# SHI-Labs/SH-GAN

Measured on AMD Instinct MI355X. Metric: generator images/sec, higher is better.
Workload: dtype f32

## Files before the change

include/shgan_hip.h:

```cpp
#ifndef SHGAN_HIP_H
#define SHGAN_HIP_H
#include <stddef.h>
#include <stdint.h>
#ifdef __cplusplus
extern "C" {
#endif

#define SHG_OK 0
#define SHG_ERR_ARG (-1)
#define SHG_ERR_LAUNCH (-2)
#define SHG_ERR_UNSUPPORTED (-3)

int shg_abi_version(void);
const char* shg_last_error(void);
int shg_device_info(int dev, char* buf, int buflen);

int shg_upfirdn2d_out_size(int H, int W, int fh, int fw, int upx, int upy, int downx, int downy, int padx0, int padx1,
                           int pady0, int pady1, int* OH, int* OW);
int shg_upfirdn2d_f32(const float* x, const float* f, float* y, int N, int C, int H, int W, int fh, int fw, int upx, int upy,
                      int downx, int downy, int padx0, int padx1, int pady0, int pady1, int flip, float gain, void* stream);
int shg_upfirdn2d_strided(const void* x, const float* f, void* y, int dtype, int N, int C, int H, int W, const long* x_strides,
                          const long* y_strides, int fh, int fw, long f_stride_y, long f_stride_x, int upx, int upy, int downx, int downy,
                          int padx0, int padx1, int pady0, int pady1, int flip, float gain, void* stream);
int shg_upfirdn2d_epilogue_f32(const float* x, const float* f, float* y, int N, int C, int H, int W, int fh, int fw, int upx,
// ... 4 lines not shown
int shg_bias_act_f32(const float* x, float* y, const float* scale, const float* bias, const float* noise, int noise_mode,
                     float noise_strength, const float* residual, int N, int C, int HW, int act, float alpha, float gain,
                     float clamp, void* stream);
int shg_bias_act_backward_f32(const float* g, const float* y, float* dx, long total, int act, float alpha, float gain, float clamp,
                              void* stream);
int shg_fma_f32(const float* a, const float* b, const float* c, float* y, long total, void* stream);
int shg_fma_bcast(const void* a, const void* b, const void* c, void* y, int nd, const long* shape, const long* sa, const long* sb,
                  const long* sc, int f64, void* stream);
int shg_mul_reduce(const void* g, const void* b, void* out, int nd, int nk, const long* shape, const long* sg, const long* sb,
                   int inner_kept, int f64, void* stream);
int shg_scale_channels_f32(const float* x, const float* s, float* y, int NC, int HW, void* stream);
int shg_sum_partials_f32(const float* part, float* out, int N, int B, int K, void* stream);
int shg_scale_cast_f32_f16(const void* src, void* dst, long n, float gain, int to_half, void* stream);
int shg_planes_to_image_f32(const float* mid, const float* bias, float* y, int N, int C, int H, int W, int lo, int OH, int OW,
                            void* stream);

int shg_conv_weight_prep_f32(const float* w, float* wt, float* wscale, float* wsq, int O, int I, int KH, int KW, int OP,
                             int demod, float gain, int flip, void* stream);
int shg_conv2d_f32(const float* x, const float* wt, float* y, int NB, int I, int O, int OP, int H, int W, int kh, int kw,
                   int mode, int pad, int wgroups, long wstride, const float* in_scale, const float* out_scale,
                   const float* bias, const float* noise, int noise_mode, float noise_strength, int act, float alpha, float gain,
                   float clamp, const float* residual, int out_mode, void* workspace, size_t ws_bytes, void* stream);
size_t shg_conv2d_workspace_bytes(int NB, int I, int O, int H, int W, int kh, int kw, int mode, int pad, int wgroups);
int shg_conv_wino_chunk(void);
int shg_conv_weight_prep_wino_f32(const float* w, const float* wscale, float* wu, int O, int I, int OP, int flip, void* stream);
int shg_conv2d_wino_f32(const float* x, const float* wu, float* y, int NB, int I, int O, int OP, int H, int W,
                        const float* in_scale, const float* out_scale, const float* bias, const float* noise, int noise_mode,
                        float noise_strength, int act, float alpha, float gain, float clamp, const float* residual, void* stream);
size_t shg_conv2d_wino_workspace_bytes(int NB, int I, int O, int OP, int H, int W);
int shg_conv2d_wino_ws_f32(const float* x, const float* wu, float* y, int NB, int I, int O, int OP, int H, int W,
                           const float* in_scale, const float* out_scale, const float* bias, const float* noise, int noise_mode,
                           float noise_strength, int act, float alpha, float gain, float clamp, const float* residual, void* workspace,
                           size_t ws_bytes, void* stream);
long shg_conv_wino4_weight_elems(int OP, int I);
int shg_conv_weight_prep_wino4_f32(const float* w, const float* wscale, float* wu, int O, int I, int OP, int flip, void* stream);
int shg_conv2d_wino4_supported(int NB, int I, int O, int H, int W);
int shg_conv2d_wino4_f32(const float* x, const float* wu, float* y, int NB, int I, int O, int OP, int H, int W,
                         const float* in_scale, const float* out_scale, const float* bias, const float* noise, int noise_mode,
                         float noise_strength, int act, float alpha, float gain, float clamp, const float* residual, void* stream);
size_t shg_conv2d_wino4_workspace_bytes(int NB, int I, int O, int OP, int H, int W);
int shg_conv2d_wino4_ws_f32(const float* x, const float* wu, float* y, int NB, int I, int O, int OP, int H, int W,
                            const float* in_scale, const float* out_scale, const float* bias, const float* noise, int noise_mode,
                            float noise_strength, int act, float alpha, float gain, float clamp, const float* residual, void* workspace,
                            size_t ws_bytes, void* stream);
int shg_upfir_planar_f32(const float* mid, const float* f, float* y, int N, int C, int H, int W, int flip, float gain,
                         const float* scale, const float* bias, const float* noise, int noise_mode, float noise_strength,
// ... 163 lines not shown
```

sh-gan_amd/_lib.py:

```python
import ctypes
import os

import torch

_HERE = os.path.dirname(os.path.abspath(__file__))
LIB_PATH = os.path.join(_HERE, 'lib', 'libshgan_hip.so')
ABI_VERSION = 40

c_fp = ctypes.c_void_p
c_i = ctypes.c_int
c_f = ctypes.c_float
c_l = ctypes.c_long
c_pp = ctypes.POINTER(ctypes.c_void_p)



class DenseGroup(ctypes.Structure):
    _fields_ = [('x1', c_fp), ('x2', c_fp), ('w', c_fp), ('b', c_fp), ('y', c_fp),
                ('ld1', c_i), ('ld2', c_i), ('K1', c_i), ('K2', c_i), ('O', c_i), ('ldy', c_i),
                ('wgain', c_f), ('bgain', c_f)]


class StyleGroup(ctypes.Structure):
    _fields_ = [('styles', c_fp), ('wsq', c_fp), ('s_out', c_fp), ('dcoef', c_fp),
# ... 5 lines not shown
        (n, c_i) for n in ('I', 'H', 'W', 'x_ctot', 'x_coff', 'O', 'kh', 'kw', 'sh', 'sw', 'ph', 'pw', 'OH', 'OW', 'y_ctot', 'y_coff', 'splitk')]


_SIGS = {
    'shg_abi_version': [],
    'shg_device_info': [c_i, ctypes.c_char_p, c_i],
    'shg_upfirdn2d_out_size': [c_i] * 12 + [ctypes.POINTER(c_i), ctypes.POINTER(c_i)],
    'shg_upfirdn2d_f32': [c_fp, c_fp, c_fp] + [c_i] * 15 + [c_f, c_fp],
    'shg_upfirdn2d_strided': [c_fp, c_fp, c_fp, c_i, c_i, c_i, c_i, c_i, ctypes.POINTER(c_l), ctypes.POINTER(c_l), c_i, c_i, c_l, c_l] + [c_i] * 9
                             + [c_f, c_fp],
    'shg_upfirdn2d_epilogue_f32': [c_fp, c_fp, c_fp] + [c_i] * 15 + [c_f, c_fp, c_fp, c_fp, c_i, c_f, c_i, c_f, c_f, c_f, c_fp, c_fp],
    'shg_bias_act_f32': [c_fp, c_fp, c_fp, c_fp, c_fp, c_i, c_f, c_fp, c_i, c_i, c_i, c_i, c_f, c_f, c_f, c_fp],
    'shg_fma_f32': [c_fp, c_fp, c_fp, c_fp, c_l, c_fp],
    'shg_fma_bcast': [c_fp, c_fp, c_fp, c_fp, c_i] + [ctypes.POINTER(c_l)] * 4 + [c_i, c_fp],
    'shg_mul_reduce': [c_fp, c_fp, c_fp, c_i, c_i] + [ctypes.POINTER(c_l)] * 3 + [c_i, c_i, c_fp],
    'shg_scale_channels_f32': [c_fp, c_fp, c_fp, c_i, c_i, c_fp],
    'shg_sum_partials_f32': [c_fp, c_fp, c_i, c_i, c_i, c_fp],
    'shg_scale_cast_f32_f16': [c_fp, c_fp, c_l, c_f, c_i, c_fp],
    'shg_planes_to_image_f32': [c_fp, c_fp, c_fp, c_i, c_i, c_i, c_i, c_i, c_i, c_i, c_fp],
    'shg_conv_weight_prep_f32': [c_fp, c_fp, c_fp, c_fp, c_i, c_i, c_i, c_i, c_i, c_i, c_f, c_i, c_fp],
    'shg_conv2d_f32': [c_fp, c_fp, c_fp] + [c_i] * 11 + [c_l, c_fp, c_fp, c_fp, c_fp, c_i, c_f, c_i, c_f, c_f, c_f, c_fp, c_i,
                       c_fp, ctypes.c_size_t, c_fp],
    'shg_conv2d_workspace_bytes': [c_i] * 10,
    'shg_conv_wino_chunk': [],
    'shg_conv_weight_prep_wino_f32': [c_fp, c_fp, c_fp, c_i, c_i, c_i, c_i, c_fp],
    'shg_conv2d_wino_f32': [c_fp, c_fp, c_fp] + [c_i] * 6 + [c_fp, c_fp, c_fp, c_fp, c_i, c_f, c_i, c_f, c_f, c_f, c_fp, c_fp],
    'shg_conv2d_wino_ws_f32': [c_fp, c_fp, c_fp] + [c_i] * 6 + [c_fp, c_fp, c_fp, c_fp, c_i, c_f, c_i, c_f, c_f, c_f, c_fp, c_fp, ctypes.c_size_t, c_fp],
    'shg_conv2d_wino_workspace_bytes': [c_i] * 6,
    'shg_conv_wino4_weight_elems': [c_i, c_i],
    'shg_conv_weight_prep_wino4_f32': [c_fp, c_fp, c_fp, c_i, c_i, c_i, c_i, c_fp],
    'shg_conv2d_wino4_supported': [c_i] * 5,
    'shg_conv2d_wino4_f32': [c_fp, c_fp, c_fp] + [c_i] * 6 + [c_fp, c_fp, c_fp, c_fp, c_i, c_f, c_i, c_f, c_f, c_f, c_fp, c_fp],
    'shg_conv2d_wino4_ws_f32': [c_fp, c_fp, c_fp] + [c_i] * 6 + [c_fp, c_fp, c_fp, c_fp, c_i, c_f, c_i, c_f, c_f, c_f, c_fp, c_fp, ctypes.c_size_t, c_fp],
    'shg_conv2d_wino4_workspace_bytes': [c_i] * 6,
    'shg_upfir_planar_f32': [c_fp, c_fp, c_fp, c_i, c_i, c_i, c_i, c_i, c_f, c_fp, c_fp, c_fp, c_i, c_f, c_i, c_f, c_f, c_f, c_fp, c_fp],
    'shg_upfir_planar_sep_supported': [c_i, c_i],
    'shg_upfir_planar_sep_f32': [c_fp, ctypes.POINTER(c_f), c_fp, c_i, c_i, c_i, c_i, c_i, c_f, c_fp, c_fp, c_fp, c_i, c_f, c_i, c_f, c_f, c_f, c_fp, c_fp],
    'shg_conv1x1_thin_in_f32': [c_fp, c_fp, c_fp, c_fp, c_i, c_i, c_i, c_i, c_f, c_i, c_f, c_f, c_f, c_fp],
    'shg_torgb_f32': [c_fp, c_fp, c_fp, c_fp, c_fp, c_fp, c_fp, c_i, c_i, c_i, c_i, c_i, c_fp],
    'shg_dense_f32': [c_fp, c_fp, c_fp, c_fp, c_i, c_i, c_i, c_i, c_i, c_f, c_f, c_i, c_f, c_f, c_f, c_fp],
    'shg_demod_weight_f32': [c_fp, c_fp, c_fp, c_fp, c_i, c_i, c_i, c_i, c_fp],
    'shg_demod_weight_backward_f32': [c_fp, c_fp, c_fp, c_fp, c_fp, c_i, c_i, c_i, c_fp],
    'shg_style_factors_f32': [c_fp, c_fp, c_fp, c_fp, c_fp, c_i, c_i, c_i, c_i, c_fp],
    'shg_style_factors_backward_f32': [c_fp, c_fp, c_fp, c_fp, c_fp, c_fp, c_fp, c_fp, c_fp, c_i, c_i, c_i, c_i, c_fp],
    'shg_matmul_nn_f32': [c_fp, c_fp, c_fp, c_i, c_i, c_i, c_i, c_i, c_f, c_fp],
    'shg_matmul_tn_f32': [c_fp, c_fp, c_fp, c_fp, c_i, c_i, c_i, c_i, c_i, c_f, c_f, c_fp],
# ... 124 lines not shown
```

sh-gan_amd/csrc/conv_mfma.hip:

```cpp
#include "shg_device.h"
#include <stdlib.h>
#include <utility>

struct ConvParams {
    const float* x;
    const float* wt;
    float* y;
    float* part;
    const float* in_scale;
    const float* out_scale;
    const float* bias;
    const float* noise;
    const float* residual;
    int NB, I, O, OP;
    int IPK;
    int H, W;
    int OHp, OWp;
    int OHt, OWt;
    int S;
    int dy0, dx0;
    int span_y, span_x;
    struct TileClass {
        int n_tiles;
        int TW, TH, TN;
        int tiles_x, tiles_y;
        int oy_base, ox_base, rows, cols;
        int PH, PW, PATCH;
    } cls[3];
    int patch_max, tn_max;
    int n_ptiles, n_otiles;
    int wgroups;
    long wstride;
    int ksplit, i_per_slice;
    long part_stride;
    int out_mode;
    int noise_mode;
    float noise_strength;
    int act;
    float alpha, gain, clamp;
    int tap_off[9];
    int tail_first, tail_ks, tail_ips, fix;
    float* tail_ws;
    int raw_reduce;
};

template <class F, int... S>
__device__ __forceinline__ void static_for_impl(F&& f, std::integer_sequence<int, S...>) {
    (f(std::integral_constant<int, S>{}), ...);
}
template <int N, class F>
__device__ __forceinline__ void static_for(F&& f) {
    static_for_impl(static_cast<F&&>(f), std::make_integer_sequence<int, N>{});
}

__device__ __forceinline__ float conv_epilogue(const ConvParams& p, float v, int n, int o, long idx, float nz) {
    if (p.out_scale) v *= p.out_scale[n * p.O + o];
    v += nz;
    if (p.bias) v += p.bias[o];
    v = p.act ? shg_lrelu_agc(v, p.alpha, p.gain, p.clamp) : v * p.gain;
    if (p.residual) v += p.residual[idx];
    return v;
}

template <int NTAPS, int KC, int MO, int NP, int WO, int WP, int XQ, bool UP, bool DB, int OCC>
__global__ __launch_bounds__(WO * WP * 64, OCC) void conv_mfma_kernel(const ConvParams p) {
    constexpr int BO = MO * 32 * WO;
    constexpr int NT = WO * WP * 64;
    constexpr int ROWS = KC * NTAPS;
    constexpr int XP = KC + 1;
    constexpr int NPH = UP ? 4 : 1;
    constexpr int V4 = ROWS * BO / 4;
    constexpr int PER = (V4 + NT - 1) / NT;
    extern __shared__ __attribute__((aligned(16))) float smem[];
    constexpr int WSZ = ROWS * BO;
    constexpr int NBUF = DB ? 2 : 1;
    float* Wl = smem;
    float* Sl = smem + NBUF * WSZ;
    float* Xl = Sl + (p.in_scale ? p.tn_max * p.i_per_slice : 0);
    const int XSZ = XP * p.patch_max;

    const int tid = threadIdx.x;
    const int lane = tid & 63, wave = tid >> 6;
    const int l31 = lane & 31, half = lane >> 5;
    const int wo = wave / WP, wp = wave % WP;

    const int nwork = p.n_ptiles * p.n_otiles;
    int kslice, work, tslice = -1;
    if (p.fix) { kslice = 0; work = p.tail_first + blockIdx.x; }
// ... 95 lines not shown
                const int ic = g * 4 + c;
                xv[k][ic] = p.x[xo[k] + (unsigned)(min(i0 + ic, p.I - 1) * HW)];
            }
        }
    };
    auto piece_store = [&](int j, int i0, int buf) __attribute__((always_inline)) {
        if (j < PW0) {
            const int e = tid + j * NT;
            if (e < V4) *reinterpret_cast<f32x4*>(Wl + buf * WSZ + e * 4) = wv[j];
        } else {
            const int k = (j - PW0) / XG, g = (j - PW0) % XG;
            const int q = tid + k * NT;
            f32x4 sc = {1.f, 1.f, 1.f, 1.f};
            if (p.in_scale) sc = *reinterpret_cast<const f32x4*>(Sl + xsn[k] + (i0 - i_begin) + g * 4);
            if (q < PATCH) {
                float* dst = Xl + buf * XSZ + q * XP + g * 4;
#pragma unroll
                for (int c = 0; c < 4; ++c)
                    dst[c] = (xoff[k] >= 0 && i0 + g * 4 + c < i_end) ? xv[k][g * 4 + c] * sc[c] : 0.f;
            }
        }
    };

    auto w_dma = [&](int i0, int buf) __attribute__((always_inline)) {
#pragma unroll
        for (int k = 0; k < PER; ++k) {
            if ((k + 1) * NT <= V4 || k * NT + wave * 64 < V4)
                __builtin_amdgcn_global_load_lds((const __attribute__((address_space(1))) void*)(wbase + (size_t)i0 * NTAPS * 64 + wl[k]),
                                                 (__attribute__((address_space(3))) void*)(Wl + buf * WSZ + (k * NT + wave * 64) * 4), 16, 0, 0);
        }
    };
    if (!p.fix) {
        if (WDMA) w_dma(i_begin, 0);
#pragma unroll
        for (int j = 0; j < NPIECE; ++j) piece_load(j, i_begin);
        __syncthreads();
#pragma unroll
        for (int j = 0; j < NPIECE; ++j) piece_store(j, i_begin, 0);
        if (DB && i_begin + KC < i_end) {
#pragma unroll
            for (int j = 0; j < NPIECE; ++j) piece_load(j, i_begin + KC);
        }
        __syncthreads();
    }

    int cur = 0;
    for (int i0 = i_begin; i0 < i_end; i0 += KC, cur ^= (DB ? 1 : 0)) {
        const bool more = i0 + KC < i_end;
        const bool more2 = i0 + 2 * KC < i_end;
        if (WDMA && more) w_dma(i0 + KC, cur ^ 1);
        if (!DB && more) {
#pragma unroll
            for (int j = 0; j < NPIECE; ++j) piece_load(j, i0 + KC);
        }
        const float* wa_c = wa + cur * WSZ;
        const float* xb_c[NP];
#pragma unroll
        for (int np = 0; np < NP; ++np) xb_c[np] = xbase[np] + cur * XSZ;
        auto handover = [&]() __attribute__((always_inline)) {
            if (more) {
#pragma unroll
                for (int j = 0; j < NPIECE; ++j) piece_store(j, i0 + KC, cur ^ 1);
            }
            if (more2) {
#pragma unroll
                for (int j = 0; j < NPIECE; ++j) piece_load(j, i0 + 2 * KC);
            }
        };
        constexpr int NGRP = (DB && WO * WP >= 8) ? (WO * WP) / 4 : 1;
        const int grp = wave >> 2;

        if constexpr (!UP) {
            constexpr int NSTEP = NTAPS * (KC / 2);
            float a[2][MO], b[2][NP];
            auto fetch = [&](int step, int buf) __attribute__((always_inline)) {
                const int t = step / (KC / 2), c2 = step % (KC / 2);
                const int toff = p.tap_off[t] * XP;
#pragma unroll
                for (int mo = 0; mo < MO; ++mo) a[buf][mo] = wa_c[((c2 * 2) * NTAPS + t) * BO + mo * 32];
#pragma unroll
                for (int np = 0; np < NP; ++np) b[buf][np] = xb_c[np][toff + c2 * 2];
            };
            fetch(0, 0);
            auto step_body = [&](int step) __attribute__((always_inline)) {
                if (step + 1 < NSTEP) fetch(step + 1, (step + 1) & 1);
                __builtin_amdgcn_sched_barrier(0);
#pragma unroll
                for (int mo = 0; mo < MO; ++mo)
#pragma unroll
                    for (int np = 0; np < NP; ++np)
// ... 47 lines not shown
#pragma unroll
                        for (int np = 0; np < NP; ++np)
                            acc[PHASE[t]][mo][np] = __builtin_amdgcn_mfma_f32_32x32x2f32(
                                a[slot & 1][tt][mo], b[c2 & 1][SHIFT[t]][np], acc[PHASE[t]][mo][np], 0, 0, 0);
                }
            };
            static_for<NSLOT>([&](auto sc) __attribute__((always_inline)) {
                constexpr int slot = decltype(sc)::value;
                slot_body(slot);
                if constexpr (DB) {
                    static_for<NGRP>([&](auto gc) __attribute__((always_inline)) {
                        constexpr int g = decltype(gc)::value;
                        if constexpr (slot == ((2 * g + 1) * NSLOT) / (2 * NGRP)) {
                            __builtin_amdgcn_sched_barrier(0);
                            if (NGRP == 1 || grp == g) handover();
                            __builtin_amdgcn_sched_barrier(0);
                        }
                    });
                }
            });
        }
        __syncthreads();
        if (!DB && more) {
#pragma unroll
            for (int j = 0; j < NPIECE; ++j) piece_store(j, i0 + KC, 0);
            __syncthreads();
        }
    }

    constexpr int NREG = NPH * MO * NP * 16;
    float* const tws = (tslice >= 0 || p.fix)
        ? p.tail_ws + ((size_t)(work - p.tail_first) * p.tail_ks + (tslice >= 0 ? tslice : 0)) * NREG * NT + tid : nullptr;

#pragma unroll
    for (int np = 0; np < NP; ++np) {
        const int j = (wp * NP + np) * 32 + l31;
        const int tn = j / THW;
        const int rem = j - tn * THW;
        const int ty = rem / TW, tx = rem - ty * TW;
        const int n = n0 + tn, oy = oy0 + ty, ox = ox0 + tx;
        if (tn >= TN || n >= p.NB || oy >= oy_end || ox >= ox_end) continue;
#pragma unroll
        for (int ph = 0; ph < NPH; ++ph) {
            long plane = (long)p.OHt * p.OWt;
            long base;
            int pix;
            if constexpr (UP) {
                const int a = ph >> 1, b = ph & 1;
// ... 45 lines not shown
                        if (o < p.O) p.y[base + (long)o * plane] = acc[ph][mo][np][r] * p.gain;
                    }
                    continue;
                }
                float osc[16], bs[16], rs[16];
#pragma unroll
                for (int r = 0; r < 16; ++r) {
                    const int o = min(ob + (r & 3) + 8 * (r >> 2), p.O - 1);
                    osc[r] = p.out_scale ? p.out_scale[n * p.O + o] : 1.f;
                    bs[r] = p.bias ? p.bias[o] : 0.f;
                    rs[r] = p.residual ? p.residual[base + (long)o * plane] : 0.f;
                }
#pragma unroll
                for (int r = 0; r < 16; ++r) {
                    const int o = ob + (r & 3) + 8 * (r >> 2);
                    if (o >= p.O) continue;
                    float v = acc[ph][mo][np][r] * osc[r] + nz + bs[r];
                    v = p.act ? shg_lrelu_agc(v, p.alpha, p.gain, p.clamp) : v * p.gain;
                    p.y[base + (long)o * plane] = v + rs[r];
                }
            }
        }
    }
}

__global__ __launch_bounds__(256) void splitk_reduce_kernel(const ConvParams p, long total, long plane) {
    const long stride = (long)gridDim.x * 256;
    for (long e = (long)blockIdx.x * 256 + threadIdx.x; e < total; e += stride) {
        float v = 0.f;
        for (int s = 0; s < p.ksplit; ++s) v += p.part[(long)s * p.part_stride + e];
        if (p.raw_reduce) { p.y[e] = v; continue; }
        const long no = e / plane;
        const int pix = (int)(e - no * plane);
        const int n = (int)(no / p.O), o = (int)(no - (long)n * p.O);
        float nz = 0.f;
        if (p.noise_mode == 1) nz = p.noise[pix] * p.noise_strength;
        else if (p.noise_mode == 2) nz = p.noise[(long)n * plane + pix] * p.noise_strength;
        p.y[e] = conv_epilogue(p, v, n, o, e, nz);
    }
}



static void tile_search(ConvParams::TileClass& t, int NB, int rows, int cols, int BP, int wgroups, int S, int span_y, int span_x,
                        int patch_cap) {
    long best = -1, bpatch = 0;
// ... 38 lines not shown
    }
    p.n_ptiles = p.cls[0].n_tiles + p.cls[1].n_tiles + p.cls[2].n_tiles;
    p.n_otiles = shg_cdiv(p.O, BO);
    p.patch_max = 0; p.tn_max = 1;
    for (int i = 0; i < 3; ++i) {
        if (p.cls[i].n_tiles == 0) continue;
        if (p.cls[i].PATCH > p.patch_max) p.patch_max = p.cls[i].PATCH;
        if (p.cls[i].TN > p.tn_max) p.tn_max = p.cls[i].TN;
    }
}

static int conv_ksplit(int grid, int chunks, bool allow) {
    int ks = 1;
    if (allow) while (grid * ks < 512 && chunks / (ks * 2) >= 4 && ks < 64) ks *= 2;
    return ks;
}

static constexpr int CONV_UP_MIN = 16;

static int conv_cu_count() { return shg_cu_count(); }

static size_t conv_tail_ws_bound(bool up) { return (size_t)256 * (up ? 128 * 128 * 4 : 128 * 256) * sizeof(float); }

template <int NTAPS, int KC, int MO, int NP, int WO, int WP, int XQ, bool UP, bool DB, int OCC>
static int launch_conv(ConvParams& p, void* workspace, size_t ws_bytes, hipStream_t s) {
    constexpr int BO = MO * 32 * WO, BP = NP * 32 * WP, NT = WO * WP * 64;
    const long out_elems = (UP && p.out_mode == 1) ? 4L * p.NB * p.O * (p.H + 1) * (p.W + 1) : (long)p.NB * p.O * p.OHt * p.OWt;
    conv_tiles(p, BO, BP, UP, XQ * NT);
    const int chunks = shg_cdiv(p.I, KC);
    int ks = conv_ksplit(p.n_ptiles * p.n_otiles, chunks, workspace != nullptr);
    if (DB && p.n_ptiles * p.n_otiles >= conv_cu_count()) ks = 1;
    while (ks > 1 && (size_t)ks * out_elems * sizeof(float) > ws_bytes) ks /= 2;
    p.i_per_slice = shg_cdiv(chunks, ks) * KC;
    p.ksplit = shg_cdiv(p.I, p.i_per_slice);
    p.raw_reduce = UP ? 1 : 0;
    p.part = p.ksplit > 1 ? (float*)workspace : nullptr;
    p.part_stride = out_elems;
    if (p.patch_max > XQ * NT) { shg_set_error("conv: patch of %d elements exceeds the staging capacity %d", p.patch_max, XQ * NT); return SHG_ERR_UNSUPPORTED; }
    if (!UP)
        for (int t = 0; t < NTAPS; ++t) {
            const int dyr = p.tap_off[t] >> 6, dxr = p.tap_off[t] & 63;
            p.tap_off[t] = dyr * p.cls[0].PW + dxr;
        }
    const size_t lds = sizeof(float) * ((DB ? 2 : 1) * ((size_t)KC * NTAPS * BO + (size_t)(KC + 1) * p.patch_max) +
                                        (p.in_scale ? (size_t)p.tn_max * p.i_per_slice : 0));
    auto kern = conv_mfma_kernel<NTAPS, KC, MO, NP, WO, WP, XQ, UP, DB, OCC>;
    if (lds > 64 * 1024) {
        if (lds > 160 * 1024) { shg_set_error("conv: LDS request %zu exceeds 160 KiB", lds); return SHG_ERR_UNSUPPORTED; }
        hipError_t e = hipFuncSetAttribute(reinterpret_cast<const void*>(kern), hipFuncAttributeMaxDynamicSharedMemorySize, (int)lds);
        if (e != hipSuccess) { shg_set_error("hipFuncSetAttribute: %s", hipGetErrorString(e)); return SHG_ERR_LAUNCH; }
    }
    const int nwork = p.n_ptiles * p.n_otiles;
    p.tail_first = nwork; p.tail_ks = 1; p.tail_ips = p.I; p.fix = 0; p.tail_ws = nullptr;
    int n_tail = 0;
    if (DB && p.ksplit == 1 && workspace) {
        const int slots = conv_cu_count();
        const int tail = nwork % slots;
        if (nwork > slots && tail > 0 && tail * 10 < slots * 6) {
            int tk = 1;
            while (tk < 8 && tail * tk * 2 <= slots && chunks / (tk * 2) >= 4) tk *= 2;
            const size_t need = (size_t)tail * tk * (BO * BP * (UP ? 4 : 1)) * sizeof(float);
            if (tk > 1 && need <= ws_bytes) {
                n_tail = tail; p.tail_first = nwork - tail; p.tail_ks = tk; p.tail_ips = shg_cdiv(chunks, tk) * KC;
                p.tail_ws = (float*)workspace;
            }
        }
    }
    const int grid = p.ksplit > 1 ? nwork * p.ksplit : p.tail_first + n_tail * p.tail_ks;
    hipLaunchKernelGGL(kern, dim3(grid), dim3(NT), lds, s, p);
// ... 233 lines not shown
        const size_t split = ks > 1 ? (size_t)ks * 4 * NB * O * (H + 1) * (W + 1) * sizeof(float) : 0;
        const size_t tail = big ? conv_tail_ws_bound(true) : 0;
        return split > tail ? split : tail;
    }
    const int S = mode == 0 ? 1 : 2;
    const int OH = (H + 2 * pad - kh) / S + 1, OW = (W + 2 * pad - kw) / S + 1;
    if (OH < 1 || OW < 1) return 0;
    const bool narrow = O <= 64;
    const int KC = kh * kw == 9 ? 8 : 32;
    const int xq = kh * kw == 1 ? 1 : (S == 1 ? 2 : (narrow ? 5 : 3));
    p.OHp = OH; p.OWp = OW; p.S = S; p.span_y = kh; p.span_x = kw;
    conv_tiles(p, narrow ? 64 : 128, narrow ? 256 : 128, false, xq * 256);
    int ks = conv_ksplit(p.n_ptiles * p.n_otiles, shg_cdiv(I, KC), true);
    if (kh * kw == 9 && !narrow && OW >= 32 && OH >= 8) {
        ConvParams q = p;
        conv_tiles(q, 128, 256, false, xq * 256);
        const int ks2 = conv_ksplit(q.n_ptiles * q.n_otiles, shg_cdiv(I, KC), true);
        if (ks2 > ks) ks = ks2;
    }
    if (ks > 1) return (size_t)ks * NB * O * OH * OW * sizeof(float);
    return (kh * kw == 9 && !narrow && OW >= 32 && OH >= 8) ? conv_tail_ws_bound(false) : 0;
}


__global__ __launch_bounds__(256) void weight_scale_kernel(const float* w, float* scale, int IK, int demod, float gain) {
    const int o = blockIdx.x;
    float acc = 0.f;
    if (demod) {
        for (int k = threadIdx.x; k < IK; k += 256) { const float v = w[(long)o * IK + k]; acc += v * v; }
        __shared__ float red[256];
        red[threadIdx.x] = acc;
        __syncthreads();
        for (int st = 128; st > 0; st >>= 1) {
            if (threadIdx.x < st) red[threadIdx.x] += red[threadIdx.x + st];
            __syncthreads();
        }
        acc = red[0];
    }
    if (threadIdx.x == 0) scale[o] = demod ? gain * rsqrtf(acc / (float)IK) : gain;
}

__global__ __launch_bounds__(256) void weight_transpose_kernel(const float* w, const float* scale, float* wt, int O, int I,
                                                               int IP, int KK, int OP, int flip) {
    __shared__ float tile[32][33];
    const int IK = I * KK;
    const int IPK = IP * KK;
// ... 45 lines not shown
```

sh-gan_amd/kernels.py:

```python
import contextlib
import ctypes
import math

import torch

from . import _lib
from ._lib import check

SQRT2 = math.sqrt(2.0)
_NULLCTX = contextlib.nullcontext()


class _Launch:
    __slots__ = ('dev', 'keep', '_ctx')

    def __init__(self):
        self.dev = None
        self.keep = []
        self._ctx = None

    def _own(self, t, name):
        if self.dev is None:
            self.dev = t.device
        elif t.device != self.dev:
            raise _lib.ShgError(f'{name} lives on {t.device}, the other operands of this call on {self.dev}')
# ... 638 lines not shown
        ws_bytes = int(lib.shg_conv2d_workspace_bytes(nb, i, pw.o, h, w, pw.kh, pw.kw, mode, pad, pw.groups))
        if ws_bytes:
            ws = L.new((ws_bytes // 4,))
    pix = (h * w) if mode == MODE_UP2T else (oh * ow)
    with _timed(L, _CONV_CLASS[mode] if pw.kh == 3 else 'conv_mfma_1x1', 2.0 * nb * pw.o * i * pw.kh * pw.kw * pix):
        check(lib.shg_conv2d_f32(
            _ptr(x), _ptr(pw.wt), _ptr(y), nb, i, pw.o, pw.op, h, w, pw.kh, pw.kw, mode, pad, pw.groups, pw.wt.shape[1],
            _ptr(in_scale), _ptr(out_scale), _ptr(bias), _ptr(noise), nmode, float(noise_strength), a, al, g, cl, _ptr(residual),
            1 if planar else 0, _ptr(ws), ws_bytes, L.stream()), 'conv2d')
    return y


DOWN_POLY_MIN_I, DOWN_POLY_MIN_OUT = 128, 32


def down_poly_supported(x, pw, force=False):
    n, i, h, w = x.shape
    if not force and (i < DOWN_POLY_MIN_I or min(h, w) // 2 < DOWN_POLY_MIN_OUT):
        return False
    return bool(DOWN_POLY and pw.groups == 1 and pw.kh == 3 and pw.kw == 3 and pw._w is not None and h % 2 == 0 and w % 2 == 0
                and x.is_cuda and _lib.get_lib().shg_conv2d_down_poly_supported(n, i, pw.o, h // 2, w // 2))


def fir_conv_down2(x, f, pw, bias=None, act=False, gain=1.0, alpha=0.2, act_gain=SQRT2, clamp=256.0, residual=None, flip_filter=False):
    L = _Launch()
    x, f = L.req(x, 'x'), L.req(f, 'f')
    if tuple(f.shape) != (4, 4):
        raise _lib.ShgError('fir_conv_down2: f must be 4x4')
    n, i, h, w = x.shape
    oh, ow = h // 2, w // 2
    lib = _lib.get_lib()
    pp4 = (ow + 1 + 3) // 4 * 4
    taps = sep_taps(f) if lib.shg_fir_pad2_sep_supported(h, w, pp4) else None
    pp = (ow + 1 + 31) // 32 * 32 if (taps is not None and w % 256 == 0) else pp4
    wa, wb = pw.down_poly()
    L.view(wa, 'weights')
    xp = L.new((4, n, i, oh + 1, pp))
    y = L.new((n, pw.o, oh, ow))
    bias, residual = L.req(bias, 'bias'), L.req(residual, 'residual')
    if residual is not None and tuple(residual.shape) != tuple(y.shape):
        raise _lib.ShgError('fir_conv_down2: residual shape mismatch')
    a, al, g, cl = _act_args(act, gain, alpha, act_gain, clamp)
    with _timed(L, 'upfirdn2d', 4.0 * (x.numel() + n * i * (h + 1) * (w + 1))):
        if taps is not None:
            check(lib.shg_fir_pad2_sep_f32(_ptr(x), taps, _ptr(xp), n, i, h, w, pp, int(bool(flip_filter)), 1.0, L.stream()), 'fir_pad2_sep')
        else:
# ... 361 lines not shown
```

sh-gan_amd/model_zoo/stylegan.py:

```python
import math

import os

import numpy as np
import torch
import torch.nn as nn

from .. import kernels
from .common import utils
from .common.get_model import get_model, register
from .stylegan_utils import grad_ops, conv2d_gradfix, conv2d_resample, fma, misc, upfirdn2d

version = '0'
symbol = 'stylegan'



def _make_act(activation):
    return None if activation is None else utils.get_unit()(activation)()


def _act_kwargs(act_obj, gain=1.0):
    if act_obj is None:
        return dict(act=False, gain=gain)
# ... 534 lines not shown
            y = self._forward_half_infer(x, gain)
            if y is not None:
                return y
        if route != 'f32_fused':
            return self._forward_train(x, gain)
        ak = _act_kwargs(self.activation, gain)
        b = self.bias.detach() if self.bias is not None else None
        k = self.weight.shape[2]
        fusable = ak is not None and self.up == 1 and self.down in (1, 2) and k in (1, 3)
        if fusable and self.down == 2 and not (k == 3 and self.resample_filter is not None and self.resample_filter.ndim == 2):
            fusable = False
        if fusable:
            if self.down == 1:
                if k == 1 and self.weight.shape[1] <= 8 and (x.shape[2] * x.shape[3]) % 4 == 0:
                    return kernels.conv1x1_thin_in(x, self.weight.detach().reshape(self.weight.shape[0], -1), b,
                                                   wgain=self.weight_gain, **ak)
                return kernels.conv2d(x, self.prepped(), mode=kernels.MODE_SAME, pad=self.padding, bias=b, **ak)
            f = self.resample_filter
            fw, fh = f.shape[1], f.shape[0]
            p = self.padding
            pads = [p + (fw - 1) // 2, p + (fw - 2) // 2, p + (fh - 1) // 2, p + (fh - 2) // 2]
            if tuple(f.shape) == (4, 4) and p == 1 and kernels.down_poly_supported(x, self.prepped()):
                return kernels.fir_conv_down2(x, f, self.prepped(), bias=b, **ak)
            y = kernels.upfirdn2d(x, f, padx0=pads[0], padx1=pads[1], pady0=pads[2], pady1=pads[3])
            return kernels.conv2d(y, self.prepped(), mode=kernels.MODE_DOWN2, pad=0, bias=b, **ak)
        w = self.weight.detach() * self.weight_gain
        y = conv2d_resample.conv2d_resample(x=x, w=w, f=self.resample_filter, up=self.up, down=self.down,
                                            padding=self.padding, flip_weight=(self.up == 1))
        if ak is None:
            if b is not None:
                y = kernels.bias_act(y, bias=b, act=False)
            return self.activation(y, gain=gain)
        return kernels.bias_act(y, bias=b, **ak)

    def __repr__(self):
        return self.repr


class synthesis_layer(conv2d_layer):

    def __init__(self, in_channels, out_channels, kernel_size, w_dim, resolution, bias=True,
                 activation='lrelu_agc(alpha=0.2, gain=sqrt_2)', up=1, resample_filter=[1, 3, 3, 1], use_noise=True):
        super().__init__(in_channels, out_channels, kernel_size, bias=bias, activation=activation, up=up, down=1,
                         resample_filter=resample_filter)
        self.affine = dense(w_dim, in_channels, bias=True, bias_init=1, activation=None)
        self.resolution = resolution
# ... 371 lines not shown
```

Baseline: 830.2.

## Fuse separable FIR pre-filter into stride-2 MFMA conv input staging

Adds a FIR variant of the MFMA conv kernel. It DMAs a raw input window into LDS and applies the separable 4x4 blur in registers while building the conv input tile, which removes the separate upfirdn2d pass and its intermediate tensor for down-sampling 3x3 convs. The path is enabled by default (env flag) for layers with few input channels and wide outputs where the polyphase path doesn't apply. In exchange it uses more LDS per block and does extra ALU work in the staging step, which may lower occupancy.

```diff
diff --git a/include/shgan_hip.h b/include/shgan_hip.h
--- a/include/shgan_hip.h
+++ b/include/shgan_hip.h
@@ -50,6 +50,10 @@
                    const float* bias, const float* noise, int noise_mode, float noise_strength, int act, float alpha, float gain,
                    float clamp, const float* residual, int out_mode, void* workspace, size_t ws_bytes, void* stream);
 size_t shg_conv2d_workspace_bytes(int NB, int I, int O, int H, int W, int kh, int kw, int mode, int pad, int wgroups);
+int shg_fir_conv2d_down_direct_supported(int NB, int I, int O, int H, int W);
+int shg_fir_conv2d_down_direct_f32(const float* x, const float* taps_host, const float* wt, float* y, int NB, int I, int O, int OP,
+                                   int H, int W, int flip, const float* bias, int act, float alpha, float gain, float clamp,
+                                   const float* residual, void* workspace, size_t ws_bytes, void* stream);
 int shg_conv_wino_chunk(void);
 int shg_conv_weight_prep_wino_f32(const float* w, const float* wscale, float* wu, int O, int I, int OP, int flip, void* stream);
 int shg_conv2d_wino_f32(const float* x, const float* wu, float* y, int NB, int I, int O, int OP, int H, int W,
diff --git a/sh-gan_amd/_lib.py b/sh-gan_amd/_lib.py
--- a/sh-gan_amd/_lib.py
+++ b/sh-gan_amd/_lib.py
@@ -51,6 +51,9 @@
     'shg_conv2d_f32': [c_fp, c_fp, c_fp] + [c_i] * 11 + [c_l, c_fp, c_fp, c_fp, c_fp, c_i, c_f, c_i, c_f, c_f, c_f, c_fp, c_i,
                        c_fp, ctypes.c_size_t, c_fp],
     'shg_conv2d_workspace_bytes': [c_i] * 10,
+    'shg_fir_conv2d_down_direct_supported': [c_i] * 5,
+    'shg_fir_conv2d_down_direct_f32': [c_fp, ctypes.POINTER(c_f), c_fp, c_fp] + [c_i] * 7 + [c_fp, c_i, c_f, c_f, c_f, c_fp, c_fp,
+                                       ctypes.c_size_t, c_fp],
     'shg_conv_wino_chunk': [],
     'shg_conv_weight_prep_wino_f32': [c_fp, c_fp, c_fp, c_i, c_i, c_i, c_i, c_fp],
     'shg_conv2d_wino_f32': [c_fp, c_fp, c_fp] + [c_i] * 6 + [c_fp, c_fp, c_fp, c_fp, c_i, c_f, c_i, c_f, c_f, c_f, c_fp, c_fp],
diff --git a/sh-gan_amd/csrc/conv_mfma.hip b/sh-gan_amd/csrc/conv_mfma.hip
--- a/sh-gan_amd/csrc/conv_mfma.hip
+++ b/sh-gan_amd/csrc/conv_mfma.hip
@@ -42,6 +42,8 @@
     int tail_first, tail_ks, tail_ips, fix;
     float* tail_ws;
     int raw_reduce;
+    float fa[4], fb[4];
+    int fir_rh, fir_rp, fir_ppu, fir_uq, fir_wreg;
 };
 
 template <class F, int... S>
@@ -62,8 +64,8 @@
     return v;
 }
 
-template <int NTAPS, int KC, int MO, int NP, int WO, int WP, int XQ, bool UP, bool DB, int OCC>
-__global__ __launch_bounds__(WO * WP * 64, OCC) void conv_mfma_kernel(const ConvParams p) {
+template <int NTAPS, int KC, int MO, int NP, int WO, int WP, int XQ, bool UP, bool DB, int OCC, bool FIR>
+__device__ __forceinline__ void conv_mfma_body(const ConvParams& p) {
     constexpr int BO = MO * 32 * WO;
     constexpr int NT = WO * WP * 64;
     constexpr int ROWS = KC * NTAPS;
@@ -205,6 +207,87 @@
         }
     };
 
+    constexpr int NW = WO * WP;
+    constexpr int RQ = FIR ? (DB ? 4 : 16) : 1;
+    float* const Rw = Xl + ((NBUF * XSZ + 3) & ~3) + wave * p.fir_wreg;
+    const int ry0 = 2 * oy0 - 2, rx0 = 2 * ox0 - 2, rxs = rx0 & ~3;
+    unsigned rsrc[RQ];
+    int rch[RQ];
+    if constexpr (FIR) {
+        const int rp4 = p.fir_rp >> 2;
+#pragma unroll
+        for (int k = 0; k < RQ; ++k) {
+            const int L = lane + 64 * k;
+            const int us = L / p.fir_ppu, pc = L - us * p.fir_ppu;
+            const int row = pc / rp4, x4 = pc - row * rp4;
+            const int u = wave + us * NW;
+            const int c = u / TN, tn = u - c * TN;
+            const int iy = ry0 + row, ix = rxs + 4 * x4, n = n0 + tn;
+            const bool ok = us < p.fir_uq && c < KC && n < p.NB && iy >= 0 && iy < p.H && ix >= 0 && ix < p.W;
+            rsrc[k] = ok ? (unsigned)(n * p.I * HW + iy * p.W + ix) : 0u;
+            rch[k] = ok ? c : 0;
+        }
+    }
+    auto raw_dma = [&](int i0) __attribute__((always_inline)) {
+#pragma unroll
+        for (int k = 0; k < RQ; ++k) {
+            if (k * 256 < p.fir_wreg)
+                __builtin_amdgcn_global_load_lds((const __attribute__((address_space(1))) void*)(p.x + rsrc[k] + (unsigned)(min(i0 + rch[k], p.I - 1) * HW)),
+                                                 (__attribute__((address_space(3))) void*)(Rw + k * 256), 16, 0, 0);
+        }
+    };
+    auto fir_store = [&](int i0, int buf) __attribute__((always_inline)) {
+        asm volatile("s_waitcnt vmcnt(0)" ::: "memory");
+        const float a0 = p.fa[0], a1 = p.fa[1], a2 = p.fa[2], a3 = p.fa[3];
+        const float b0 = p.fb[0], b1 = p.fb[1], b2 = p.fb[2], b3 = p.fb[3];
+        for (int us = 0; us < p.fir_uq; ++us) {
+            const int u = wave + us * NW;
+            const int c = u / TN, tn = u - c * TN;
+            if (c >= KC) break;
+            const bool uok = n0 + tn < p.NB && i0 + c < i_end;
+            for (int col = lane; col < PW_; col += 64) {
+                const float* src = Rw + us * p.fir_ppu * 4 + (rx0 - rxs) + col;
+                float* dst = Xl + buf * XSZ + (tn * PHW + col) * XP + c;
+                const int ix = rx0 + col;
+                const bool m0 = uok && ix >= 0 && ix < p.W, m1 = uok && ix + 1 >= 0 && ix + 1 < p.W;
+                const bool m2 = uok && ix + 2 >= 0 && ix + 2 < p.W, m3 = uok && ix + 3 >= 0 && ix + 3 < p.W;
+                float h[4] = {0.f, 0.f, 0.f, 0.f};
+                auto row_step = [&](auto J, int rr) __attribute__((always_inline)) {
+                    constexpr int j = decltype(J)::value;
+                    if (rr < p.fir_rh) {
+                        const int iy = ry0 + rr;
+                        const bool rok = iy >= 0 && iy < p.H;
+                        const float* s = src + rr * p.fir_rp;
+                        const float v0 = s[0], v1 = s[1], v2 = s[2], v3 = s[3];
+                        const float s2 = (rok && m0) ? v0 : 0.f, s1 = (rok && m1) ? v1 : 0.f;
+                        const float cc = (rok && m2) ? v2 : 0.f, n1 = (rok && m3) ? v3 : 0.f;
+                        h[j] = a0 * s2 + a1 * s1 + a2 * cc + a3 * n1;
+                        if (rr >= 3) {
+                            constexpr int j0 = (j + 1) & 3, j1 = (j + 2) & 3, j2 = (j + 3) & 3;
+                            dst[(rr - 3) * PW_ * XP] = b0 * h[j0] + b1 * h[j1] + b2 * h[j2] + b3 * h[j];
+                        }
+                    }
+                };
+                for (int r = 0; r < p.fir_rh; r += 4) {
+                    row_step(std::integral_constant<int, 0>{}, r);
+                    row_step(std::integral_constant<int, 1>{}, r + 1);
+                    row_step(std::integral_constant<int, 2>{}, r + 2);
+                    row_step(std::integral_constant<int, 3>{}, r + 3);
+                }
+            }
+        }
+    };
+    auto stage_load = [&](int i0) __attribute__((always_inline)) {
+#pragma unroll
+        for (int j = 0; j < (FIR ? PW0 : NPIECE); ++j) piece_load(j, i0);
+        if constexpr (FIR) raw_dma(i0);
+    };
+    auto stage_store = [&](int i0, int buf) __attribute__((always_inline)) {
+#pragma unroll
+        for (int j = 0; j < (FIR ? PW0 : NPIECE); ++j) piece_store(j, i0, buf);
+        if constexpr (FIR) fir_store(i0, buf);
+    };
+
     auto w_dma = [&](int i0, int buf) __attribute__((always_inline)) {
 #pragma unroll
         for (int k = 0; k < PER; ++k) {
@@ -215,15 +298,10 @@
     };
     if (!p.fix) {
         if (WDMA) w_dma(i_begin, 0);
-#pragma unroll
-        for (int j = 0; j < NPIECE; ++j) piece_load(j, i_begin);
+        stage_load(i_begin);
         __syncthreads();
-#pragma unroll
-        for (int j = 0; j < NPIECE; ++j) piece_store(j, i_begin, 0);
-        if (DB && i_begin + KC < i_end) {
-#pragma unroll
-            for (int j = 0; j < NPIECE; ++j) piece_load(j, i_begin + KC);
-        }
+        stage_store(i_begin, 0);
+        if (DB && i_begin + KC < i_end) stage_load(i_begin + KC);
         __syncthreads();
     }
 
@@ -232,23 +310,14 @@
         const bool more = i0 + KC < i_end;
         const bool more2 = i0 + 2 * KC < i_end;
         if (WDMA && more) w_dma(i0 + KC, cur ^ 1);
-        if (!DB && more) {
-#pragma unroll
-            for (int j = 0; j < NPIECE; ++j) piece_load(j, i0 + KC);
-        }
+        if (!DB && more) stage_load(i0 + KC);
         const float* wa_c = wa + cur * WSZ;
         const float* xb_c[NP];
 #pragma unroll
         for (int np = 0; np < NP; ++np) xb_c[np] = xbase[np] + cur * XSZ;
         auto handover = [&]() __attribute__((always_inline)) {
-            if (more) {
-#pragma unroll
-                for (int j = 0; j < NPIECE; ++j) piece_store(j, i0 + KC, cur ^ 1);
-            }
-            if (more2) {
-#pragma unroll
-                for (int j = 0; j < NPIECE; ++j) piece_load(j, i0 + 2 * KC);
-            }
+            if (more) stage_store(i0 + KC, cur ^ 1);
+            if (more2) stage_load(i0 + 2 * KC);
         };
         constexpr int NGRP = (DB && WO * WP >= 8) ? (WO * WP) / 4 : 1;
         const int grp = wave >> 2;
@@ -342,8 +411,7 @@
         }
         __syncthreads();
         if (!DB && more) {
-#pragma unroll
-            for (int j = 0; j < NPIECE; ++j) piece_store(j, i0 + KC, 0);
+            stage_store(i0 + KC, 0);
             __syncthreads();
         }
     }
@@ -435,6 +503,17 @@
             }
         }
     }
+}
+
+template <int NTAPS, int KC, int MO, int NP, int WO, int WP, int XQ, bool UP, bool DB, int OCC>
+__global__ __launch_bounds__(WO * WP * 64, OCC) void conv_mfma_kernel(const ConvParams p) {
+    conv_mfma_body<NTAPS, KC, MO, NP, WO, WP, XQ, UP, DB, OCC, false>(p);
+}
+
+template <int NTAPS, int KC, int MO, int NP, int WO, int WP, int XQ, bool UP, bool DB, int OCC>
+__global__ __launch_bounds__(WO * WP * 64, OCC) void conv_mfma_kernel_fir(const ConvParams p) {
+    static_assert(NTAPS == 9 && !UP, "FIR pre-filter: stride-2 tap-list instantiations");
+    conv_mfma_body<NTAPS, KC, MO, NP, WO, WP, XQ, UP, DB, OCC, true>(p);
 }
 
 __global__ __launch_bounds__(256) void splitk_reduce_kernel(const ConvParams p, long total, long plane) {
@@ -519,8 +598,8 @@
 
 static size_t conv_tail_ws_bound(bool up) { return (size_t)256 * (up ? 128 * 128 * 4 : 128 * 256) * sizeof(float); }
 
-template <int NTAPS, int KC, int MO, int NP, int WO, int WP, int XQ, bool UP, bool DB, int OCC>
-static int launch_conv(ConvParams& p, void* workspace, size_t ws_bytes, hipStream_t s) {
+template <int NTAPS, int KC, int MO, int NP, int WO, int WP, int XQ, bool UP, bool DB, int OCC, bool FIR = false>
+static int launch_conv(ConvParams& p, void* workspace, size_t ws_bytes, hipStream_t s, bool dry = false) {
     constexpr int BO = MO * 32 * WO, BP = NP * 32 * WP, NT = WO * WP * 64;
     const long out_elems = (UP && p.out_mode == 1) ? 4L * p.NB * p.O * (p.H + 1) * (p.W + 1) : (long)p.NB * p.O * p.OHt * p.OWt;
     conv_tiles(p, BO, BP, UP, XQ * NT);
@@ -539,9 +618,23 @@
             const int dyr = p.tap_off[t] >> 6, dxr = p.tap_off[t] & 63;
             p.tap_off[t] = dyr * p.cls[0].PW + dxr;
         }
-    const size_t lds = sizeof(float) * ((DB ? 2 : 1) * ((size_t)KC * NTAPS * BO + (size_t)(KC + 1) * p.patch_max) +
-                                        (p.in_scale ? (size_t)p.tn_max * p.i_per_slice : 0));
-    auto kern = conv_mfma_kernel<NTAPS, KC, MO, NP, WO, WP, XQ, UP, DB, OCC>;
+    size_t lds = sizeof(float) * ((DB ? 2 : 1) * ((size_t)KC * NTAPS * BO + (size_t)(KC + 1) * p.patch_max) +
+                                  (p.in_scale ? (size_t)p.tn_max * p.i_per_slice : 0));
+    void (*kern)(const ConvParams);
+    if constexpr (FIR) kern = conv_mfma_kernel_fir<NTAPS, KC, MO, NP, WO, WP, XQ, UP, DB, OCC>;
+    else kern = conv_mfma_kernel<NTAPS, KC, MO, NP, WO, WP, XQ, UP, DB, OCC>;
+    if constexpr (FIR) {
+        constexpr int NW = WO * WP, RQ = DB ? 4 : 16;
+        const ConvParams::TileClass& t = p.cls[0];
+        p.fir_rh = t.PH + 3; p.fir_rp = (t.PW + 3 + 2 + 3) / 4 * 4; p.fir_ppu = p.fir_rh * (p.fir_rp / 4);
+        p.fir_uq = shg_cdiv(KC * t.TN, NW);
+        const int pieces = shg_cdiv(p.fir_uq * p.fir_ppu, 64) * 64;
+        p.fir_wreg = pieces * 4;
+        if (pieces > RQ * 64) { shg_set_error("fir_conv: raw window of %d pieces per wave exceeds the staging capacity %d", pieces, RQ * 64); return SHG_ERR_UNSUPPORTED; }
+        lds = sizeof(float) * ((DB ? 2 : 1) * (size_t)KC * NTAPS * BO + (((DB ? 2 : 1) * (size_t)(KC + 1) * p.patch_max + 3) & ~(size_t)3) +
+                               (size_t)NW * p.fir_wreg);
+    }
+    if (dry) return lds <= 160 * 1024 ? SHG_OK : SHG_ERR_UNSUPPORTED;
     if (lds > 64 * 1024) {
         if (lds > 160 * 1024) { shg_set_error("conv: LDS request %zu exceeds 160 KiB", lds); return SHG_ERR_UNSUPPORTED; }
         hipError_t e = hipFuncSetAttribute(reinterpret_cast<const void*>(kern), hipFuncAttributeMaxDynamicSharedMemorySize, (int)lds);
@@ -821,6 +914,50 @@
     return (kh * kw == 9 && !narrow && OW >= 32 && OH >= 8) ? conv_tail_ws_bound(false) : 0;
 }
 
+extern "C" int shg_fir_pad2_sep_supported(int H, int W, int PP);
+
+static int conv_fir_dispatch(ConvParams& p, void* workspace, size_t ws_bytes, hipStream_t s, bool dry) {
+    const bool narrow = p.O <= 64;
+    if (!narrow && p.OWp >= 32 && p.OHp >= 8)
+        return launch_conv<9, 8, 1, 2, 4, 2, 2, false, true, 2, true>(p, workspace, ws_bytes, s, dry);
+    return narrow ? launch_conv<9, 8, 2, 2, 1, 4, 5, false, false, 2, true>(p, workspace, ws_bytes, s, dry)
+                  : launch_conv<9, 8, 2, 2, 2, 2, 3, false, false, 2, true>(p, workspace, ws_bytes, s, dry);
+}
+
+static int conv_fir_fill(ConvParams& p, const float* x, const float* wt, float* y, int NB, int I, int O, int OP, int H, int W,
+                         const float* bias, int act, float alpha, float gain, float clamp, const float* residual) {
+    int rc = conv_fill(p, x, wt, y, NB, I, O, OP, H + 1, W + 1, 3, 3, 1, 0, 1, 0, nullptr, nullptr, bias, nullptr, 0, 0.f, act, alpha, gain,
+                       clamp, residual, 0);
+    if (rc != SHG_OK) return rc;
+    p.H = H; p.W = W;
+    return SHG_OK;
+}
+
+extern "C" int shg_fir_conv2d_down_direct_supported(int NB, int I, int O, int H, int W) {
+    if (NB < 1 || I < 1 || O < 1 || H < 4 || W < 8 || H % 2 || W % 4 || !shg_fir_pad2_sep_supported(H, W, 0)) return 0;
+    if ((long)NB * I * (H + 1) * (W + 1) >= 2147483647L) return 0;
+    static float dummy;
+    ConvParams p;
+    if (conv_fir_fill(p, &dummy, &dummy, &dummy, NB, I, O, (O + 63) / 64 * 64, H, W, nullptr, 0, 0.f, 1.f, -1.f, nullptr) != SHG_OK) return 0;
+    return conv_fir_dispatch(p, nullptr, 0, nullptr, true) == SHG_OK;
+}
+
+extern "C" int shg_fir_conv2d_down_direct_f32(const float* x, const float* taps_host, const float* wt, float* y, int NB, int I, int O, int OP,
+                                              int H, int W, int flip, const float* bias, int act, float alpha, float gain, float clamp,
+                                              const float* residual, void* workspace, size_t ws_bytes, void* stream) {
+    SHG_CHECK_ARG(taps_host, "fir_conv2d_down_direct: null pointer");
+    SHG_CHECK_ARG(shg_fir_conv2d_down_direct_supported(NB, I, O, H, W), "fir_conv2d_down_direct: unsupported geometry (shg_fir_conv2d_down_direct_supported)");
+    SHG_CHECK_ARG((reinterpret_cast<uintptr_t>(x) & 15) == 0, "fir_conv2d_down_direct: x must be 16-byte aligned");
+    ConvParams p;
+    int rc = conv_fir_fill(p, x, wt, y, NB, I, O, OP, H, W, bias, act, alpha, gain, clamp, residual);
+    if (rc != SHG_OK) return rc;
+    for (int k = 0; k < 4; ++k) {
+        p.fa[k] = taps_host[flip ? k : 3 - k];
+        p.fb[k] = taps_host[4 + (flip ? k : 3 - k)];
+    }
+    return conv_fir_dispatch(p, workspace, ws_bytes, (hipStream_t)stream, false);
+}
+
 
 __global__ __launch_bounds__(256) void weight_scale_kernel(const float* w, float* scale, int IK, int demod, float gain) {
     const int o = blockIdx.x;
diff --git a/sh-gan_amd/kernels.py b/sh-gan_amd/kernels.py
--- a/sh-gan_amd/kernels.py
+++ b/sh-gan_amd/kernels.py
@@ -1,6 +1,7 @@
 import contextlib
 import ctypes
 import math
+import os
 
 import torch
 
@@ -685,6 +686,45 @@
                 and x.is_cuda and _lib.get_lib().shg_conv2d_down_poly_supported(n, i, pw.o, h // 2, w // 2))
 
 
+FUSE_DOWN_FIR = os.environ.get('SHG_FUSE_DOWN_FIR', '1') == '1'
+DOWN_FUSE_MIN_O, DOWN_FUSE_MIN_OH, DOWN_FUSE_MIN_OW = 65, 8, 32
+
+
+def down_direct_fused_supported(x, f, pw, force=False):
+    n, i, h, w = x.shape
+    if not force and not (FUSE_DOWN_FIR and i < DOWN_POLY_MIN_I and pw.o >= DOWN_FUSE_MIN_O and h // 2 >= DOWN_FUSE_MIN_OH
+                          and w // 2 >= DOWN_FUSE_MIN_OW):
+        return False
+    return bool(pw.groups == 1 and pw.kh == 3 and pw.kw == 3 and x.is_cuda and x.dtype == torch.float32 and x.is_contiguous()
+                and x.data_ptr() % 16 == 0 and f is not None and tuple(f.shape) == (4, 4) and h % 2 == 0 and w % 2 == 0
+                and _lib.get_lib().shg_fir_conv2d_down_direct_supported(n, i, pw.o, h, w) and sep_taps(f) is not None)
+
+
+def fir_conv_down_direct(x, f, pw, bias=None, act=False, gain=1.0, alpha=0.2, act_gain=SQRT2, clamp=256.0, residual=None, flip_filter=False):
+    L = _Launch()
+    x, f = L.req(x, 'x'), L.req(f, 'f')
+    taps = sep_taps(f)
+    if taps is None:
+        raise _lib.ShgError('fir_conv_down_direct: f must be a separable 4x4 filter')
+    n, i, h, w = x.shape
+    oh, ow = h // 2, w // 2
+    lib = _lib.get_lib()
+    L.view(pw.wt, 'weights')
+    y = L.new((n, pw.o, oh, ow))
+    bias, residual = L.req(bias, 'bias'), L.req(residual, 'residual')
+    if residual is not None and tuple(residual.shape) != tuple(y.shape):
+        raise _lib.ShgError('fir_conv_down_direct: residual shape mismatch')
+    a, al, g, cl = _act_args(act, gain, alpha, act_gain, clamp)
+    ws, ws_bytes = None, int(lib.shg_conv2d_workspace_bytes(n, i, pw.o, h + 1, w + 1, 3, 3, MODE_DOWN2, 0, 1))
+    if ws_bytes:
+        ws = L.new((ws_bytes // 4,))
+    with _timed(L, _CONV_CLASS[MODE_DOWN2], 2.0 * n * pw.o * i * 9 * oh * ow):
+        check(lib.shg_fir_conv2d_down_direct_f32(_ptr(x), taps, _ptr(pw.wt), _ptr(y), n, i, pw.o, pw.op, h, w, int(bool(flip_filter)),
+                                                 _ptr(bias), a, al, g, cl, _ptr(residual), _ptr(ws), ws_bytes, L.stream()),
+              'fir_conv2d_down_direct')
+    return y
+
+
 def fir_conv_down2(x, f, pw, bias=None, act=False, gain=1.0, alpha=0.2, act_gain=SQRT2, clamp=256.0, residual=None, flip_filter=False):
     L = _Launch()
     x, f = L.req(x, 'x'), L.req(f, 'f')
diff --git a/sh-gan_amd/model_zoo/stylegan.py b/sh-gan_amd/model_zoo/stylegan.py
--- a/sh-gan_amd/model_zoo/stylegan.py
+++ b/sh-gan_amd/model_zoo/stylegan.py
@@ -580,6 +580,8 @@
             pads = [p + (fw - 1) // 2, p + (fw - 2) // 2, p + (fh - 1) // 2, p + (fh - 2) // 2]
             if tuple(f.shape) == (4, 4) and p == 1 and kernels.down_poly_supported(x, self.prepped()):
                 return kernels.fir_conv_down2(x, f, self.prepped(), bias=b, **ak)
+            if tuple(f.shape) == (4, 4) and p == 1 and kernels.down_direct_fused_supported(x, f, self.prepped()):
+                return kernels.fir_conv_down_direct(x, f, self.prepped(), bias=b, **ak)
             y = kernels.upfirdn2d(x, f, padx0=pads[0], padx1=pads[1], pady0=pads[2], pady1=pads[3])
             return kernels.conv2d(y, self.prepped(), mode=kernels.MODE_DOWN2, pad=0, bias=b, **ak)
         w = self.weight.detach() * self.weight_gain
```

New measurement: 807.9. 0.973x the previous value.
